# alexanderswerdlow/BEVGen

Hardware: AMD Instinct MI355X
Metric: multi-view scenes/sec (6x256x256) (higher is better)
Workload: dtype f32 (GEMM/conv/attention products as 3 f16 MFMAs on hi/lo splits, fp32 accumulate); 1 GPU; BASELINE configs[1]: Route M MaskGit, 6x256x256, batch 16 scenes/GPU, 18 iterations, + VQGAN decode to uint8; global_batch=16, parallelism=scene-parallel x1 (RCCL gather of uint8 pixels), precision_mode=f16x3

## Files before the change

### bevgen_amd/_lib.py

```python
from __future__ import annotations

import ctypes as C
import os
from typing import Optional

_HERE = os.path.dirname(os.path.abspath(__file__))
LIB_PATH = os.environ.get("BEVGEN_LIB_PATH") or os.path.join(_HERE, "csrc", "libbevgen_hip.so")
HEADER_PATH = os.path.join(os.path.dirname(_HERE), "include", "bevgen_hip.h")

ABI_VERSION = 10
ROUTE_MASKGIT, ROUTE_AR = 0, 1
PRECISION_FP32, PRECISION_BF16, PRECISION_F16X3, PRECISION_F16X1 = 0, 1, 2, 3
KV_F32, KV_F16 = 0, 1
DECODE_FUSED, DECODE_PER_OP, DECODE_SPLIT, DECODE_AUTO = 0, 1, 2, 3
VQ_OUT_RAW, VQ_OUT_DENORM, VQ_OUT_U8 = 0, 1, 2
W_F32, W_F16 = 0, 1
DTYPE_F32, DTYPE_I64, DTYPE_U8, DTYPE_F64 = 0, 1, 2, 3
ERR_NUMERIC = -5
STATUS_MLP_BARRIER, STATUS_MLP_PLACEMENT, STATUS_NONFINITE_LOGITS, STATUS_F16_RANGE, STATUS_NONFINITE_PIXELS, STATUS_NONFINITE_LATENTS = 1, 2, 4, 8, 16, 32


class BevgenError(RuntimeError):
    def __init__(self, code: int, message: str):
        super().__init__(f"libbevgen_hip error {code}: {message}")
# ... 15 lines not shown


_p = C.c_void_p
_i = C.c_int
_f = C.c_float
_l = C.c_long

SIGNATURES = {
    "bevgen_create": (_i, [C.POINTER(bevgen_cfg), _i, C.POINTER(_p)]),
    "bevgen_destroy": (None, [_p]),
    "bevgen_last_error": (C.c_char_p, [_p]),
    "bevgen_abi_version": (_i, []),
    "bevgen_synchronize": (_i, [_p, _p]),
    "bevgen_status": (_i, [_p, C.POINTER(C.c_uint)]),
    "bevgen_load_tensor": (_i, [_p, C.c_char_p, _p, _i, _i, C.POINTER(C.c_int64)]),
    "bevgen_set_tables": (_i, [_p, _p, _p, _p, _p, _p]),
    "bevgen_finalize": (_i, [_p]),
    "bevgen_muse_forward": (_i, [_p, _p, _p, _p, _p, _i, _p, _p, _p]),
    "bevgen_maskgit_generate": (_i, [_p, _p, _p, _p, _i, _i, C.POINTER(C.c_int32), _f, _i, _f, _p, _p, _p, _p, C.c_uint64, _p]),
    "bevgen_maskgit_generate_ex": (_i, [_p, _p, _p, _p, _i, _i, C.POINTER(C.c_int32), _f, _i, _f, _p, _p, _p, _p, C.c_uint64, _i, _i, _p]),
    "bevgen_op_philox_uniform": (_i, [_p, C.c_uint64, C.c_uint, C.c_uint, _i, _l, _p, _p]),
    "bevgen_sparse_self_attention": (_i, [_p, _p, _p, _p, _p, _p, _p, _i, _i, _i, _i, _p, _p]),
    "bevgen_ar_prefill": (_i, [_p, _p, _p, _p, _i, _p]),
    "bevgen_ar_logits": (_i, [_p, _p, _p]),
    "bevgen_ar_decode_step": (_i, [_p, _p, _p]),
    "bevgen_ar_forward": (_i, [_p, _p, _p, _p, _i, _p, _i, _p, _p, _p, _p, _p, _p]),
    "bevgen_ar_sample": (_i, [_p, _p, _p, _p, _i, _i, _i, _f, _i, _p, _i, _p, _p, _p]),
    "bevgen_ar_sample_forced": (_i, [_p, _p, _p, _p, _i, _i, _i, _f, _i, _p, _i, _p, _p, _p, _p]),
    "bevgen_vq_decode": (_i, [_p, _p, _i, _i, _i, _i, _p, _p]),
    "bevgen_vq_decode_latents": (_i, [_p, _p, _i, _i, _i, _i, _p, _p]),
    "bevgen_vq_encode": (_i, [_p, _p, _i, _i, _i, _p, _p]),
    "bevgen_vq_range_exponents": (_i, [_p, C.POINTER(C.c_int32), _i, C.POINTER(_i)]),
    "bevgen_op_gemm": (_i, [_p, _p, _p, _p, _p, _p, _i, _i, _i, _i, _i, _p]),
    "bevgen_op_ln_gemm": (_i, [_p, _p, _p, _p, _f, _p, _p, _p, _i, _i, _i, _i, _i, C.POINTER(_i), _p]),
    "bevgen_op_mlp_fused": (_i, [_p, _p, _p, _p, _f, _p, _p, _p, _p, _i, _p, _i, _i, _p]),
    "bevgen_op_remask": (_i, [_p, _p, _p, _p, _i, _i, _i, C.c_int64, _p]),
    "bevgen_op_maskgit_pick": (_i, [_p, _p, _p, _i, _p, _i, _i, _i, _f, C.c_int64, C.c_uint64, C.c_uint, _p, _i, _p]),
    "bevgen_op_critic_scores": (_i, [_p, _p, _i, _p, _p, _p, _f, _f, C.c_uint64, C.c_uint, _p, _i, _i, _p]),
    "bevgen_op_ar_pick": (_i, [_p, _p, _i, _p, _p, _p, _p, _i, _i, _i, _f, _p, _p, _i, _p, _p, _p, _p, _i, _i, _i, _i, _p]),
    "bevgen_op_ar_score_rows": (_i, [_p, _p, _i, _p, _p, _p, _i, _i, _i, _i, _i, _p, _p, _p]),
    "bevgen_op_mean_fixed_order": (_i, [_p, _p, _l, _p, _p]),
    "bevgen_op_layernorm": (_i, [_p, _p, _p, _p, _p, _i, _i, _f, _p]),
    "bevgen_op_geglu_layernorm": (_i, [_p, _p, _p, _p, _i, _i, _i, _p]),
    "bevgen_op_attention": (_i, [_p, _p, _p, _p, _p, _i, _i, _i, _i, _i, _f, _p, _p]),
    "bevgen_op_attention_ex": (_i, [_p, _p, _p, _p, _p, _i, _i, _i, _i, _i, _f, _i, _p, _p]),
    "bevgen_op_decode_attention": (_i, [_p, _p, _p, _p, _i, _p, _i, _p, _i, _l, _i, _i, _i, _i, _f, _p, _p]),
    "bevgen_op_ar_attn_fused": (_i, [_p, _p, _p, _i, _p, _p, _p, _p, _p, _i, _p, _p, _i, _p, _i, _p, _p, _i, _i, _i, _i, _i, _i, _i, _i, _p, _p]),
    "bevgen_op_conv3x3": (_i, [_p, _p, _p, _p, _p, _p, _i, _i, _i, _i, _i, _i, _p]),
    "bevgen_op_groupnorm": (_i, [_p, _p, _p, _p, _p, _i, _i, _i, _i, _p]),
    "bevgen_op_range_split": (_i, [_p, _p, _i, _i, _i, _p, _p, _p]),
    "bevgen_op_conv3x3_down": (_i, [_p, _p, _p, _p, _p, _i, _i, _i, _i, _i, _p]),
    "bevgen_op_vq_attn_block": (_i, [_p, _p, _p, _p, _p, _p, _p, _p, _p, _p, _p, _p, _p, _i, _i, _i, _i, _p]),
    "bevgen_op_vq_out_tail": (_i, [_p, _p, _p, _p, _p, _p, _p, _p, _i, _i, _p, _i, _i, _i, _i, _p]),
    "bevgen_op_vq_quantize": (_i, [_p, _p, _p, _p, _p, _p, _l, _i, _i, _p]),
    "bevgen_op_conv3x3_gn_stats": (_i, [_p, _p, _p, _p, _i, _p, _p, _p, _i, _i, _i, _i, _i, _p]),
    "bevgen_op_conv_ranged": (_i, [_p, _p, _p, _p, _i, _p, _p, _i, _i, _i, _i, _i, _p]),
    "bevgen_decode_attention_splits": (_i, [_i, _i, _i]),
    "bevgen_profile_begin": (_i, [_p]),
    "bevgen_profile_end": (_i, [_p, C.POINTER(C.c_double)]),
    "bevgen_ar_step_timing": (_i, [_p, _i]),
    "bevgen_ar_step_times": (_i, [_p, C.POINTER(C.c_float), _i, C.POINTER(_i)]),
    "bevgen_set_trace_buffer": (_i, [_p, _p]),
}

_lib: Optional[C.CDLL] = None

# ... 33 lines not shown
```

### bevgen_amd/csrc/api.cpp

```cpp
#include <memory>

#include "model.h"
#include "profiler.h"

using namespace bevgen;

struct bevgen_ctx : public Ctx {};

static thread_local std::string g_create_error;

template <class F>
static int guarded(bevgen_ctx* ctx, F&& f, bool check_first = true) {
    try {
        if (!ctx) return BEVGEN_ERR_INVALID;
        HIP_CHECK(hipSetDevice(ctx->device));
        split_registry_set(ctx->cfg.precision == BEVGEN_PRECISION_F16X3 ? &ctx->split : nullptr);
        struct CurrentProf {
            Profiler* old;
            unsigned* old_st;
            CurrentProf(Profiler* p, unsigned* st) : old(prof_set_current(p)), old_st(status_set_current(st)) {}
            ~CurrentProf() { prof_set_current(old); status_set_current(old_st); }
        } cur(&ctx->prof, ctx->status_dev);
        if (check_first) ctx->check_status("raised by an earlier call on this context");
        f();
// ... 260 lines not shown
            uint16_t *bp, *ap;
            ctx->arena.carve([&](Arena& ar) {
                bp = ar.get<uint16_t>((size_t)N * K * 2);
                ap = skinny >= 3 ? ar.get<uint16_t>((size_t)M * K * 2) : nullptr;
                g.kpart = skinny >= 3 && ksplit3 ? ar.get<float>((size_t)3 * M * N) : nullptr;
                g.sk_ws = skinny >= 3 && stream_k ? ar.alloc(gemm_sk_ws_bytes()) : nullptr;
            });
            launch_split_weight(w, bp, (long)N * K, (hipStream_t)stream);
            g.B_hi = bp; g.B_lo = bp + 32;
            g.a_hi_only = single;
            g.b_lo_zero = single;
            if (skinny >= 3) {
                g.b_lo_zero = skinny == 4;
                launch_split_weight(a, ap, (long)M * K, (hipStream_t)stream);
                g.A_hi = ap; g.A_lo = ap + 32;
                if (ksplit3) g.ksplit = 3;
                if (stream_k) {
                    HIP_CHECK(hipMemsetAsync(g.sk_ws, 0, 1024 * sizeof(unsigned), (hipStream_t)stream));
                    g.sk_epoch = 1; g.sk_force = true;
                }
                launch_gemm_split_glds(g, (hipStream_t)stream);
            } else {
                launch_gemm_split(g, (hipStream_t)stream);
            }
        } else if (skinny) {
            float* ws;
            ctx->arena.carve([&](Arena& ar) { ws = reinterpret_cast<float*>(ar.alloc(gemm_skinny_ws_bytes(M, N, K))); });
            launch_gemm_skinny_ws(g, ws, (hipStream_t)stream);
        }
        else launch_gemm(g, (hipStream_t)stream);
    });
}

int bevgen_op_ln_gemm(bevgen_ctx* ctx, const float* a, const float* ln_w, const float* ln_b, float eps, const float* w, const float* bias, float* c, int M, int N, int K,
                      int act_gelu, int ksplit, int* ksplit_out, void* stream) {
    return guarded(ctx, [&] {
        BG_REQUIRE(skinny_fused_supported(M, N, K, ln_w != nullptr), "op_ln_gemm: unsupported shape M=%d N=%d K=%d", M, N, K);
        SkinnyFusedArgs g;
        g.A = a; g.lda = K; g.ln_w = ln_w; g.ln_b = ln_b; g.eps = eps;
        float *wp, *cs, *ds;
        ctx->arena.carve([&](Arena& ar) {
            wp = ar.get<float>(skinny_packed_floats(N, K));
            cs = ksplit == -1 ? ar.get<float>((size_t)N) : nullptr;
            ds = ksplit == -1 ? ar.get<float>((size_t)N) : nullptr;
        });
        launch_pack_skinny_weight(w, wp, N, K, (hipStream_t)stream);
        g.Wp = wp; g.bias = bias; g.C = c; g.ldc = N;
        g.M = M; g.N = N; g.K = K; g.act = act_gelu ? ACT_GELU : ACT_NONE;
        g.ksplit = ksplit > 0 ? ksplit : (ln_w ? 1 : skinny_fused_ksplit(N, K));
        if (ksplit == -1) {
            BG_REQUIRE(ln_w && ln_b && bias, "op_ln_gemm: ksplit = -1 (folded LayerNorm) needs gamma, beta and a bias");
            launch_ar_ln_fold(w, bias, ln_w, ln_b, cs, ds, N, K, (hipStream_t)stream);
            g.ln_cs = cs; g.ln_ds = ds;
        }
        if (ksplit_out) *ksplit_out = g.ksplit;
        g.trace = ctx->trace ? ctx->trace + 4096 * 8 : nullptr;
        launch_skinny_fused(g, (hipStream_t)stream);
    });
}

int bevgen_op_mlp_fused(bevgen_ctx* ctx, const float* x, const float* ln_w, const float* ln_b, float eps, const float* w1, const float* b1, const float* w2, const float* b2,
                        int w_f16, float* out, int M, int D, void* stream) {
    return guarded(ctx, [&] {
        hipStream_t s = (hipStream_t)stream;
        BG_REQUIRE(x && ln_w && ln_b && w1 && b1 && w2 && b2 && out, "op_mlp_fused: missing operand");
        BG_REQUIRE(mlp_fused_supported(M, D, w_f16 != 0), "op_mlp_fused: unsupported shape M=%d D=%d (or a device with fewer CUs than workgroups / BEVGEN_MLP_FUSE=0)", M, D);
// ... 381 lines not shown
```

### bevgen_amd/csrc/gemm_split_glds.hip

```cpp
#include "common.h"
#include "kernels.h"
#include "profiler.h"
#include <type_traits>
#include <vector>
#include <cstdio>

namespace bevgen {

typedef _Float16 half8 __attribute__((ext_vector_type(8)));
typedef unsigned u32x4 __attribute__((ext_vector_type(4)));

struct RowDiv {
    float d, r;
    __device__ __forceinline__ explicit RowDiv(float d_) : d(d_) {
        float r0 = __builtin_amdgcn_rcpf(d_);
        const float e = fmaf(-d_, r0, 1.0f);
        r0 = fmaf(e, r0, r0);
        const float e2 = fmaf(-d_, r0, 1.0f);
        r = fmaf(e2, r0, r0);
    }
    __device__ __forceinline__ float operator()(float x) const {
        const float q0 = x * r;
        const float e = fmaf(-d, q0, x);
        return fmaf(e, r, q0);
// ... 7 lines not shown
__device__ unsigned long long g_gemm_trace[5 * 2048 * 8];
__device__ unsigned long long g_gemm_tr_tmp[2];
#define GT_STAMP(i) do { if (MODE == MODE_PLAIN && !KS) gt[i] = __builtin_amdgcn_s_memrealtime(); } while (0)
#else
#define GT_STAMP(i) do { } while (0)
#endif
constexpr float kGLoInv = 1.f / 2048.f;

__device__ __forceinline__ void glds16(const _Float16* src, _Float16* lds_wave_base) {
    __builtin_amdgcn_global_load_lds((const __attribute__((address_space(1))) void*)src, (__attribute__((address_space(3))) void*)lds_wave_base, 16, 0, 0);
}
__device__ __forceinline__ void glds16_buf(__amdgpu_buffer_rsrc_t rsrc, unsigned voff, int soff, _Float16* lds_wave_base) {
    __builtin_amdgcn_raw_ptr_buffer_load_lds(rsrc, (__attribute__((address_space(3))) void*)lds_wave_base, 16, (int)voff, soff, 0, 0);
}
template <int N>
__device__ __forceinline__ void wait_vmcnt() { asm volatile("s_waitcnt vmcnt(%0)" ::"n"(N) : "memory"); }
template <int DMA, int MAXN>
__device__ __forceinline__ void wait_tiles(int n) {
    if constexpr (MAXN <= 0) wait_vmcnt<0>();
    else {
        if (n >= MAXN) wait_vmcnt<MAXN * DMA>();
        else wait_tiles<DMA, MAXN - 1>(n);
    }
}

template <int DMA, int MAXN, int X>
__device__ __forceinline__ void wait_tiles_x(int n) {
    if constexpr (MAXN <= 0) wait_vmcnt<X>();
    else {
        if (n >= MAXN) wait_vmcnt<MAXN * DMA + X>();
        else wait_tiles_x<DMA, MAXN - 1, X>(n);
    }
}

template <int MODE, int WM, int S, bool W16, bool KS, int TI, int TJ, bool SKK = false, bool A16 = false>
__device__ __forceinline__ void gemm_tile(const GemmArgs& g, const int tx, const int ty, const int kt_first, const int nk, const int ksl, const int kz, const int sk_role,
                                          const int sk_first, const int tid
#ifdef BEVGEN_GEMM_TRACE
                                          , unsigned long long* gt
#endif
                                          ) {
    static_assert(!A16 || (W16 && MODE == MODE_PLAIN && !SKK), "single-product instantiations: rounded weight, plain GEMM, not the stream-K kernel");
    constexpr int TBM = WM * 64;
    constexpr int NW = WM * 8 / (TI * TJ);
    constexpr int WROWS = TI * 32;
    constexpr int WCOLS = TJ * 32;
    constexpr int WN = GBN / WCOLS;
    constexpr int NAJ = TBM / 8 / NW;
    constexpr int NBJ = 16 / NW;
    constexpr int AREGION = TBM * 2 * GBK;
    constexpr int STAGE_H = AREGION + GBN * 2 * GBK;
    constexpr int DMA = NAJ + NBJ;
    extern __shared__ __attribute__((aligned(1024))) _Float16 smem_g[];
    int lane = tid & 63;
    const int wave = __builtin_amdgcn_readfirstlane(tid >> 6);
    const int wm = wave / WN, wn = wave % WN;
    int r = lane & 31, h = lane >> 5;
    const int n0 = tx * GBN, m0 = ty * TBM + g.m_base;
    const int n0l = n0, m0l = m0;

    const _Float16* Ap = reinterpret_cast<const _Float16*>(g.A_hi);
    const _Float16* Bp = reinterpret_cast<const _Float16*>(g.B_hi);

    constexpr bool CONVG = MODE == MODE_CONV3, CONVS = MODE == MODE_CONV3S, CONV = CONVG || CONVS;
    unsigned a_off[NAJ], b_off[NBJ];
    int a_img[CONVG ? NAJ : 1], a_yx[CONVG ? NAJ : 1];
// ... 860 lines not shown
            if (Pp) {
                s1 += xor32(s1); s2 += xor32(s2);
                if (h == 0 && m < g.M) reinterpret_cast<float2*>(g.ln_out_stats)[(long)((n0 >> 6) + wn) * g.ln_rows + mc] = make_float2(s1, s2);
            }
        }
        if (bad) status_raise(g.status, BG_ST_F16_RANGE);
        return;
    }
    if (KS && ksl > 1) {
        float* P = g.kpart + (long)kz * g.M * g.N;
#pragma unroll
        for (int i = 0; i < TI; ++i) {
            const int m = m0 + wm * WROWS + i * 32 + r;
            if (m >= g.M) continue;
#pragma unroll
            for (int j = 0; j < 2; ++j)
#pragma unroll
                for (int qq = 0; qq < 4; ++qq) {
                    const int n = n0 + wn * 64 + j * 32 + 8 * qq + 4 * h;
#pragma unroll
                    for (int e = 0; e < 4; ++e)
                        if (n + e < g.N) P[(long)m * g.N + n + e] = accM[i][j][qq * 4 + e] + accC[i][j][qq * 4 + e] * kGLoInv;
                }
        }
        return;
    }
    }
    float* C = g.C;
    const float* Rp = g.R;
    unsigned ln_bad = 0;
    const bool vec_ok = ((g.ldc & 3) == 0) && (!Rp || (g.ldr & 3) == 0) && ((reinterpret_cast<uintptr_t>(C) & 15) == 0) &&
                        (!Rp || (reinterpret_cast<uintptr_t>(Rp) & 15) == 0);
    if constexpr (STG) {
        if (g.row_major_epi && vec_ok && (g.N & 3) == 0 && !g.ln_out_planes) {
#pragma unroll
            for (int i = 0; i < TI; ++i)
#pragma unroll
                for (int j = 0; j < TJ; ++j)
#pragma unroll
                    for (int qq = 0; qq < 4; ++qq) {
                        f32x4 v;
#pragma unroll
                        for (int e = 0; e < 4; ++e) v[e] = accM[i][j][qq * 4 + e] + accC[i][j][qq * 4 + e] * kGLoInv;
                        *reinterpret_cast<f32x4*>(pl + (i * 32 + r) * RS + j * 32 + 8 * qq + 4 * h) = v;
                    }
            constexpr int LPR = WCOLS / 4, RPP = 64 / LPR, NP = WROWS / RPP;
            const int c = lane % LPR, rr = lane / LPR;
            const int n = n0 + wn * WCOLS + 4 * c;
            const int nc = min(n, g.N - 4);
            f32x4 b4 = {0.f, 0.f, 0.f, 0.f};
            if (g.bias_n) b4 = *reinterpret_cast<const f32x4*>(g.bias_n + nc);
            f32x4 rres[NP];
            float bmr[NP];
#pragma unroll
            for (int s2 = 0; s2 < NP; ++s2) {
                const int m = min(m0 + wm * WROWS + s2 * RPP + rr, g.M - 1);
                bmr[s2] = g.bias_m ? g.bias_m[m] : 0.f;
                rres[s2] = Rp ? *reinterpret_cast<const f32x4*>(Rp + (long)m * g.ldr + nc) : f32x4{0.f, 0.f, 0.f, 0.f};
            }
#pragma unroll
            for (int s2 = 0; s2 < NP; ++s2) {
                const int row = s2 * RPP + rr, m = m0 + wm * WROWS + row;
                const f32x4 a = *reinterpret_cast<const f32x4*>(pl + row * RS + 4 * c);
                f32x4 o;
#pragma unroll
                for (int e = 0; e < 4; ++e) {
                    float t = a[e] * g.alpha + bmr[s2];
                    t += b4[e];
                    if (g.act == ACT_GELU) t = gelu_erf(t);
                    o[e] = t + rres[s2][e];
                }
                if (m < g.M && n < g.N) *reinterpret_cast<f32x4*>(C + (long)m * g.ldc + n) = o;
            }
            return;
        }
    }
    f32x4 bias4[TJ][4];
#pragma unroll
    for (int j = 0; j < TJ; ++j)
#pragma unroll
        for (int qq = 0; qq < 4; ++qq) {
            const int n = n0 + wn * WCOLS + j * 32 + 8 * qq + 4 * h;
#pragma unroll
            for (int e = 0; e < 4; ++e) bias4[j][qq][e] = (g.bias_n && n + e < g.N) ? g.bias_n[n + e] : 0.f;
        }
    f32x4 rv[TI][TJ][4];
    float bm[TI];
#pragma unroll
    for (int i = 0; i < TI; ++i) {
        const int m = min(m0 + wm * WROWS + i * 32 + r, g.M - 1);
        bm[i] = g.bias_m ? g.bias_m[m] : 0.f;
#pragma unroll
        for (int j = 0; j < TJ; ++j)
#pragma unroll
            for (int qq = 0; qq < 4; ++qq) {
                const int n = n0 + wn * WCOLS + j * 32 + 8 * qq + 4 * h;
                if (Rp && vec_ok && n + 3 < g.N) rv[i][j][qq] = *reinterpret_cast<const f32x4*>(Rp + (long)m * g.ldr + n);
                else if (Rp) {
#pragma unroll
                    for (int e = 0; e < 4; ++e) rv[i][j][qq][e] = Rp[(long)m * g.ldr + min(n + e, g.N - 1)];
                } else rv[i][j][qq] = f32x4{0.f, 0.f, 0.f, 0.f};
            }
    }
#pragma unroll
    for (int i = 0; i < TI; ++i) {
// ... 219 lines not shown
```

### bevgen_amd/csrc/muse.cpp

```cpp
#include "model.h"
#include "muse_plan.h"

namespace bevgen {

namespace {

struct MuseWs {
    int B = 0;
    int S = 1;
    bool generate = false;

    long rows = 0;
    float *img = nullptr, *c_embed = nullptr, *context = nullptr;
    int64_t* cond_g = nullptr; float* c_embed_g = nullptr;
    std::vector<float*> crossK, crossV;
    float *logits = nullptr, *scores = nullptr;
    float *x = nullptr, *xn = nullptr, *qraw = nullptr, *kvraw = nullptr, *Q = nullptr, *Ks = nullptr, *Vs = nullptr, *att = nullptr, *h = nullptr, *g = nullptr;
    size_t kvS = 0, kvC = 0;
    float* attn_ws = nullptr; int attn_ks = 1;
    float* kpart = nullptr;
    float *stats_d = nullptr, *stats_f = nullptr;
    float* rowstat = nullptr;
    void* sk_ws = nullptr;
    unsigned sk_epoch = 0;
    const float *token_emb = nullptr, *pos_emb = nullptr, *norm_g = nullptr, *to_logits = nullptr, *critic_w = nullptr, *critic_b = nullptr;
};

MuseSwitches muse_switches() {
    static const MuseSwitches once = [] {
        const auto env = [](const char* name, int dflt) { const char* v = getenv(name); return v ? atoi(v) : dflt; };
        MuseSwitches s;
        s.qkv_merge = env("BEVGEN_QKV_MERGE", 1);
        s.qkv_wm4 = env("BEVGEN_QKV_WM4", 1);
        s.ksplit = env("BEVGEN_KSPLIT", 0);
        s.attn_ksplit = env("BEVGEN_ATTN_KSPLIT", 0);
        return s;
    }();
    MuseSwitches s = once;
    const char *fold = getenv("BEVGEN_LN_FOLD"), *merge = getenv("BEVGEN_LN_MERGE");
    s.ln_fold = fold ? atoi(fold) : 1;
    s.ln_merge = merge ? (merge[0] == 't' ? 1 : 0) : -1;
    return s;
}

struct Planes { _Float16 *hi, *lo; };
Planes planes_of(float* buf, size_t n) { _Float16* hi = reinterpret_cast<_Float16*>(buf); return {hi, hi + n}; }

struct In { const float* p = nullptr; int ld = 0; };
struct Out { float* p = nullptr; int ld = 0; };

GemmArgs gemm_args(const Ctx& c, In W, Out C, int M, int N, int K, In R = {}) {
    GemmArgs g;
    g.B = W.p; g.C = C.p; g.R = R.p;
    g.M = M; g.N = N; g.K = K;
    g.ldb = W.ld; g.ldc = C.ld; g.ldr = R.ld;
    g.a_hi_only = c.single_product;
    return g;
}
void gemm(In A, GemmArgs g, hipStream_t s) {
    g.A = A.p; g.lda = A.ld;
    launch_gemm(g, s);
}
GemmArgs on_planes(const void* planes, int lda, GemmArgs g) {
    g.A_hi = reinterpret_cast<const uint16_t*>(planes); g.A_lo = g.A_hi + 32;
    g.lda = lda;
    return g;
}

struct LnFold {
    const float* in_stats = nullptr; const float* in_cs = nullptr;
    const float* in_gsums = nullptr; int in_groups = 0, in_count = 0;
    void* out_planes = nullptr; float* out_stats = nullptr; int out_ld = 0;
};
// ... 112 lines not shown
    sa.bias = c.bias_cross; sa.bias_pk = c.bias_cross_pk; sa.ldbias = c.ldC;
    sa.kv_group = w.S;
    launch_attention_split(sa, f.s);
    project(f, PROJ_OUT, on_planes(w.att, D, gemm_args(c, {l.to_out[1], D}, {w.x, D}, rows, D, D, {w.x, D})), f.fold == 2 ? &f.prod_x : nullptr);
}

void feed_forward_split(Fwd& f, const MuseLayer& l, bool last) {
    const Ctx& c = f.c;
    MuseWs& w = f.w;
    const int D = c.D, rows = f.rows, fold = f.fold;
    if (fold != 2) launch_layernorm_planes(w.x, D, l.ff_g0, nullptr, w.xn, D, rows, D, 1e-5f, f.s);
    if (l.ff_w1_geglu) {
        GemmArgs ge = on_planes(w.xn, D, gemm_args(c, {fold == 2 ? l.fold_w1 : l.ff_w1_geglu, D}, {w.h, c.Fpad}, rows, 2 * c.Fpad, D));
        ge.epi = EPI_GEGLU;
        LnFold fg;
        if (fold == 2) fg = consumer(f, w.stats_d, D / 32, D, l.fold_w1_cs);
        if (fold >= 1) { fg.out_planes = w.g; fg.out_stats = w.stats_f; fg.out_ld = c.Fpad; }
        project(f, PROJ_GEGLU, ge, fold >= 1 ? &fg : nullptr);
        if (fold == 0) launch_layernorm_planes(w.h, c.Fpad, l.ff_g3, nullptr, w.g, c.Fpad, rows, c.F, 1e-5f, f.s);
    } else {
        project(f, PROJ_UP, on_planes(w.xn, D, gemm_args(c, {l.ff_w1, D}, {w.h, 2 * c.F}, rows, 2 * c.F, D)));
        launch_geglu_layernorm_planes(w.h, 2 * c.F, l.ff_g3, w.g, c.Fpad, rows, c.F, 1e-5f, f.s);
    }
    LnFold fd;
    if (fold >= 1 && l.ff_w1_geglu) fd = consumer(f, w.stats_f, c.Fpad / 32, c.F, l.fold_w4_cs);
    const bool prod_next = fold == 2 && !last;
    if (prod_next) { fd.out_planes = w.xn; fd.out_stats = w.stats_d; fd.out_ld = D; }
    const bool cons = fd.in_stats || fd.in_gsums, any = cons || fd.out_planes;
    project(f, PROJ_OUT, on_planes(w.g, c.Fpad, gemm_args(c, {cons ? l.fold_w4 : l.ff_w4_padded, c.Fpad}, {w.x, D}, rows, D, c.Fpad, {w.x, D})), any ? &fd : nullptr);
    f.x_planes_ready = prod_next;
}

void muse_blocks_split(const Ctx& c, MuseWs& w, hipStream_t s) {
    Fwd f{c, w, s, (int)w.rows, w.B, c.N, muse_switches()};
    f.fold = muse_fold_level(f.sw, !c.muse.empty() && c.muse[0].fold_w4);
    f.tile_merge = muse_tile_merge(f.sw, f.rows);
    f.prod_x.out_planes = w.xn; f.prod_x.out_stats = w.stats_d; f.prod_x.out_ld = c.D;
    const int layers = c.cfg.num_layers;
    for (int i = 0; i < layers; ++i) {
        const MuseLayer& l = c.muse[i];
        self_attention_split(f, l);
        cross_attention_split(f, l, i);
        feed_forward_split(f, l, i + 1 == layers);
    }
}

void muse_blocks_f32(const Ctx& c, MuseWs& w, hipStream_t s) {
    const int D = c.D, H = c.H, B = w.B, N = c.N, F = c.F, Fpad = c.Fpad, rows = (int)w.rows;
    AttnArgs self{};
    self.Q = w.Q; self.K = w.Ks; self.V = w.Vs; self.bias = c.bias_self; self.R = nullptr; self.O = w.att;
    self.B = B; self.H = H; self.Nq = N; self.Nk_pad = c.NkS_pad;
    self.q_bstride = (long)H * N * 64; self.q_hstride = (long)N * 64;
    self.kv_bstride = (long)H * c.NkS_pad * 64; self.kv_hstride = (long)c.NkS_pad * 64;
    self.ldbias = c.ldS; self.bias_head_stride = 0; self.scale = 8.0f;
    self.o_bstride = (long)N * D; self.o_qstride = D; self.o_hstride = 64;
    AttnArgs cross = self;
    cross.bias = c.bias_cross; cross.Nk_pad = c.NkC_pad; cross.ldbias = c.ldC;
    cross.kv_bstride = (long)H * c.NkC_pad * 64; cross.kv_hstride = (long)c.NkC_pad * 64;
    cross.kv_group = w.S;
    for (int i = 0; i < c.cfg.num_layers; ++i) {
        const MuseLayer& l = c.muse[i];
        launch_layernorm(w.x, D, l.norm_g[0], nullptr, w.xn, D, rows, D, 1e-5f, s);
        gemm({w.xn, D}, gemm_args(c, {l.to_q[0], D}, {w.qraw, D}, rows, D, D), s);
        gemm({w.xn, D}, gemm_args(c, {l.to_kv[0], D}, {w.kvraw, 2 * D}, rows, 2 * D, D), s);
        launch_muse_q_prep(w.qraw, l.q_scale[0], w.Q, B, H, N, s);
        launch_muse_kv_prep(w.kvraw, l.null_kv[0], l.k_scale[0], w.Ks, w.Vs, B, H, N, c.NkS_pad, s);
        launch_attention(self, s);
        gemm({w.att, D}, gemm_args(c, {l.to_out[0], D}, {w.x, D}, rows, D, D, {w.x, D}), s);
        launch_layernorm(w.x, D, l.norm_g[1], nullptr, w.xn, D, rows, D, 1e-5f, s);
        gemm({w.xn, D}, gemm_args(c, {l.to_q[1], D}, {w.qraw, D}, rows, D, D), s);
        launch_muse_q_prep(w.qraw, l.q_scale[1], w.Q, B, H, N, s);
        cross.K = w.crossK[i]; cross.V = w.crossV[i];
        launch_attention(cross, s);
        gemm({w.att, D}, gemm_args(c, {l.to_out[1], D}, {w.x, D}, rows, D, D, {w.x, D}), s);
        launch_layernorm(w.x, D, l.ff_g0, nullptr, w.xn, D, rows, D, 1e-5f, s);
        gemm({w.xn, D}, gemm_args(c, {l.ff_w1, D}, {w.h, 2 * F}, rows, 2 * F, D), s);
        launch_geglu_layernorm(w.h, 2 * F, l.ff_g3, w.g, Fpad, rows, F, 1e-5f, s);
        gemm({w.g, Fpad}, gemm_args(c, {l.ff_w4_padded, Fpad}, {w.x, D}, rows, D, Fpad, {w.x, D}), s);
    }
}

void muse_layout(const Ctx& c, MuseWs& w, Arena& a) {
    const auto& g = c.cfg;
    const MuseSwitches sw = muse_switches();
    const int D = c.D, H = c.H, B = w.B, G = B / w.S;
    w.img = g.image_embed ? a.get<float>((size_t)w.rows * D) : nullptr;
    w.c_embed = g.image_embed ? a.get<float>((size_t)B * g.num_cams * D) : nullptr;
    w.context = a.get<float>((size_t)G * c.K * D);
    w.x = a.get<float>((size_t)w.rows * D);
    w.xn = a.get<float>((size_t)w.rows * D);
    w.qraw = a.get<float>((size_t)w.rows * D);
    w.att = a.get<float>((size_t)w.rows * D);
    w.kvraw = a.get<float>((size_t)std::max<long>(w.rows, (long)B * c.K) * 2 * D);
    w.Q = a.get<float>((size_t)w.rows * D);
    w.kvS = (size_t)B * H * c.NkS_pad * 64;
    w.Ks = a.get<float>(w.kvS);
    w.Vs = a.get<float>(w.kvS);
    w.h = a.get<float>((size_t)w.rows * 2 * c.F);
    w.g = a.get<float>((size_t)w.rows * c.Fpad);
    w.kpart = muse_needs_kpart(w.rows, D, c.Fpad, sw) ? a.get<float>((size_t)kMuseKsplitMax * w.rows * D) : nullptr;
    w.attn_ks = pick_attn_ksplit((long)cdiv(c.N, 256) * H * B, c.NkS_pad / 32, sw.attn_ksplit);
    w.attn_ws = w.attn_ks > 1 ? a.get<float>((size_t)attn_split_ws_floats(B, H, c.N, w.attn_ks)) : nullptr;
    w.stats_d = a.get<float>((size_t)w.rows * 2 * (D / 32));
    w.stats_f = a.get<float>((size_t)w.rows * 2 * (c.Fpad / 32));
    w.rowstat = a.get<float>((size_t)w.rows * 2);
    w.sk_ws = w.rows <= kMuseSkMaxRows && g.precision == BEVGEN_PRECISION_F16X3 ? a.alloc(gemm_sk_ws_bytes()) : nullptr;
    w.cond_g = w.S > 1 ? a.get<int64_t>((size_t)G * c.K) : nullptr;
    w.c_embed_g = w.S > 1 && g.image_embed ? a.get<float>((size_t)G * g.num_cams * D) : nullptr;
    w.kvC = (size_t)G * H * c.NkC_pad * 64;
    w.crossK.resize(g.num_layers);
    w.crossV.resize(g.num_layers);
    for (int i = 0; i < g.num_layers; ++i) {
        w.crossK[i] = a.get<float>(w.kvC);
        w.crossV[i] = a.get<float>(w.kvC);
    }
    w.logits = w.generate ? a.get<float>((size_t)w.rows * c.V) : nullptr;
    w.scores = w.generate ? a.get<float>((size_t)w.rows) : nullptr;
// ... 109 lines not shown
```

### bevgen_amd/csrc/muse_plan.h

```cpp
#pragma once
#include "gemm_plan.h"

namespace bevgen {

struct MuseSwitches {
    int ln_fold = 1;
    int ln_merge = -1;
    int qkv_merge = 1;
    int qkv_wm4 = 1;
    int ksplit = 0;
    int attn_ksplit = 0;
};

inline int muse_fold_level(const MuseSwitches& sw, bool has_fold_constants) { return has_fold_constants ? std::max(0, std::min(sw.ln_fold, 2)) : 0; }

inline bool muse_tile_merge(const MuseSwitches& sw, long rows) { return sw.ln_merge >= 0 ? sw.ln_merge == 1 : rows <= 3072; }

inline bool muse_qkv_merged(const MuseSwitches& sw, long rows) { return sw.qkv_merge != 0 && (sw.qkv_merge != 3 || rows <= 3072); }

constexpr int kMuseKsplitMax = 6;
inline int pick_ksplit(long rows, int N, int K, int ksplit_switch) {
    if ((long)cdiv(rows, 256) * cdiv(N, 128) >= 256) return 1;
    const long tiles = (long)cdiv(rows, 128) * cdiv(N, 128);
    if (tiles >= 160) return 1;
    int s = (K >= 2048 && tiles > 128) ? 2 : 1;
    if (ksplit_switch > 0) s = std::min(kMuseKsplitMax, ksplit_switch);
    while (s > 1 && K / 32 < 2 * s) --s;
    return s;
}
inline bool muse_needs_kpart(long rows, int D, int Fpad, const MuseSwitches& sw) { return std::max(pick_ksplit(rows, D, D, sw.ksplit), pick_ksplit(rows, D, Fpad, sw.ksplit)) > 1; }

inline int pick_attn_ksplit(long blocks, int ntiles, int attn_ksplit_switch) {
    if (attn_ksplit_switch > 0) return std::max(1, std::min(std::min(attn_ksplit_switch, 8), ntiles));
    if (blocks * 2 > 256) return 1;
    const int ks = std::min(std::min(4, (int)(256 / blocks)), ntiles / 8);
    return std::max(ks, 1);
}

constexpr long kMuseSkMaxRows = 8192;

enum MuseProj { PROJ_OUT = 0, PROJ_Q = 1, PROJ_KV = 2, PROJ_GEGLU = 3, PROJ_UP = 4 };
struct MuseProjIn {
    MuseProj kind = PROJ_UP;
    long M = 0; int N = 0, K = 0;
    bool fold_role = false;
    bool merged = false;
    bool has_kpart = false;
// ... 30 lines not shown
```

### bevgen_amd/runtime.py

```python
from __future__ import annotations

import ctypes as C
import os
import math
from typing import Dict, Mapping, Optional, Sequence

import numpy as np
import torch

from . import _lib, tables
from ._lib import bevgen_cfg
from .weights import ff_inner_dim


def _ptr(t: Optional[torch.Tensor]):
    return None if t is None else C.c_void_p(t.data_ptr())


def _stream(device=None):
    return C.c_void_p(torch.cuda.current_stream(device).cuda_stream)


def _req(t: torch.Tensor, dtype, device, name: str) -> torch.Tensor:
    if t.dtype != dtype:
# ... 349 lines not shown
    def profile_begin(self):
        self._check(self.lib.bevgen_profile_begin(self._h))

    def profile_end(self) -> Dict[str, Dict[str, float]]:
        buf = (C.c_double * (3 * len(self.PROFILE_KINDS)))()
        self._check(self.lib.bevgen_profile_end(self._h, buf))
        return {k: {"launches": buf[3 * i], "ms": buf[3 * i + 1], "work": buf[3 * i + 2]} for i, k in enumerate(self.PROFILE_KINDS)}

    def ar_step_timing(self, enable: bool = True):
        self._check(self.lib.bevgen_ar_step_timing(self._h, int(enable)))

    def ar_step_times(self, cap: int = 4096):
        buf = (C.c_float * cap)()
        n = C.c_int(0)
        self._check(self.lib.bevgen_ar_step_times(self._h, buf, cap, C.byref(n)))
        return np.frombuffer(buf, dtype=np.float32, count=n.value).copy()

    def trace_begin(self):
        self._trace = torch.zeros((3, 4096, 8), dtype=torch.int64, device=self.device)
        self._check(self.lib.bevgen_set_trace_buffer(self._h, _ptr(self._trace)))

    def trace_end(self):
        torch.cuda.synchronize()
        self._check(self.lib.bevgen_set_trace_buffer(self._h, None))
        return self._trace.cpu()

    def op_gemm(self, a, w, bias=None, residual=None, gelu=False, skinny=False):
        M, K = a.shape
        N = w.shape[0]
        c = torch.empty((M, N), dtype=torch.float32, device=self.device)
        self._check(self.lib.bevgen_op_gemm(self._h, _ptr(a), _ptr(w), _ptr(bias), _ptr(residual), _ptr(c), M, N, K, int(gelu), int(skinny), self._s()))
        return c

    def op_ln_gemm(self, a, w, ln_w=None, ln_b=None, bias=None, gelu=False, ksplit=0, eps=1e-5):
        M, K = a.shape
        N = w.shape[0]
        ks = C.c_int(0)
        out = torch.empty((4, M, N), dtype=torch.float32, device=self.device)
        self._check(self.lib.bevgen_op_ln_gemm(self._h, _ptr(a), _ptr(ln_w), _ptr(ln_b), float(eps), _ptr(w), _ptr(bias), _ptr(out), M, N, K, int(gelu), int(ksplit),
                                               C.byref(ks), self._s()))
        return out[0] if ks.value == 1 else out[:ks.value].sum(0)

    def op_mlp_fused(self, x, ln_w, ln_b, w1, b1, w2, b2, w_f16=False, eps=1e-5):
        M, D = x.shape
        out = torch.empty((M, D), dtype=torch.float32, device=self.device)
        self._check(self.lib.bevgen_op_mlp_fused(self._h, _ptr(x), _ptr(ln_w), _ptr(ln_b), float(eps), _ptr(w1), _ptr(b1), _ptr(w2), _ptr(b2), int(w_f16), _ptr(out), M, D, self._s()))
        return out

    @staticmethod
    def _ld(t, ld):
        assert t.dim() == 2 and (t.shape[1] == 1 or t.stride(1) == 1), "rows must be unit-stride"
        return int(ld) if ld is not None else (t.stride(0) if t.shape[0] > 1 else t.shape[1])

    def op_remask(self, ids, scores, n_mask, mask_id, init_ids=None):
        rows, T = ids.shape
        self._check(self.lib.bevgen_op_remask(self._h, _ptr(ids), _ptr(scores), _ptr(init_ids), rows, T, int(n_mask), int(mask_id), self._s()))
        return ids

    def op_maskgit_pick(self, ids, logits, V, *, mask_id, k=None, topk_filter_thres=None, temperature=1.0, gumbel_u=None, seed=0, it=0, conf_scores=None, conf_mode=0, ldl=None):
        if k is None:
            k = V if topk_filter_thres is None else topk_count(topk_filter_thres, V)
        self._check(self.lib.bevgen_op_maskgit_pick(self._h, _ptr(ids), _ptr(logits), self._ld(logits, ldl), _ptr(gumbel_u), ids.numel(), int(V), int(k), float(temperature),
                                                    int(mask_id), C.c_uint64(int(seed) & 0xFFFFFFFFFFFFFFFF), int(it), _ptr(conf_scores), int(conf_mode), self._s()))
        return ids

    def op_critic_scores(self, embed, w, b, D=None, *, u=None, noise_scale=0.0, frac=0.0, seed=0, it=0, lde=None):
# ... 149 lines not shown
```

### include/bevgen_hip.h

```cpp
#ifndef BEVGEN_HIP_H
#define BEVGEN_HIP_H

#include <stddef.h>
#include <stdint.h>

#ifdef __cplusplus
extern "C" {
#endif

#define BEVGEN_ABI_VERSION 10

enum { BEVGEN_ROUTE_MASKGIT = 0, BEVGEN_ROUTE_AR = 1 };
enum { BEVGEN_PRECISION_FP32 = 0, BEVGEN_PRECISION_BF16 = 1 , BEVGEN_PRECISION_F16X3 = 2, BEVGEN_PRECISION_F16X1 = 3 };
enum { BEVGEN_KV_F32 = 0, BEVGEN_KV_F16 = 1 };
enum { BEVGEN_DECODE_FUSED = 0, BEVGEN_DECODE_PER_OP = 1, BEVGEN_DECODE_SPLIT = 2, BEVGEN_DECODE_AUTO = 3 };
enum { BEVGEN_W_F32 = 0, BEVGEN_W_F16 = 1 };
enum { BEVGEN_DTYPE_F32 = 0, BEVGEN_DTYPE_I64 = 1, BEVGEN_DTYPE_U8 = 2, BEVGEN_DTYPE_F64 = 3 };

enum {
    BEVGEN_OK = 0,
    BEVGEN_ERR_INVALID = -1,
    BEVGEN_ERR_HIP = -2,
    BEVGEN_ERR_STATE = -3,
    BEVGEN_ERR_INTERNAL = -4,
// ... 68 lines not shown

int bevgen_sparse_self_attention(bevgen_ctx* ctx, const float* d_q, const float* d_k, const float* d_v, const int64_t* d_layout,
                                 const float* d_attn_mask, const float* d_add_mask, int B, int H, int L, int block, float* d_out, void* stream);

int bevgen_ar_prefill(bevgen_ctx* ctx, const int64_t* d_cond_ids, const float* d_I_inv, const float* d_E_inv, int B, void* stream);

int bevgen_ar_logits(bevgen_ctx* ctx, float* d_logits, void* stream);

int bevgen_ar_decode_step(bevgen_ctx* ctx, const int64_t* d_token, void* stream);

int bevgen_ar_forward(bevgen_ctx* ctx, const int64_t* d_cond_ids, const float* d_I_inv, const float* d_E_inv, int B, const int64_t* d_ids, int n_steps,
                      float* d_logits, const int64_t* d_target, const float* d_weight, float* d_nll, float* d_loss, void* stream);

int bevgen_ar_sample(bevgen_ctx* ctx, const int64_t* d_cond_ids, const float* d_I_inv, const float* d_E_inv, int B, int steps,
                     int top_k, float temperature, int greedy, const float* d_noise_u, int samples_per_layout,
                     int64_t* d_out_ids, float* d_step_logits , void* stream);

int bevgen_ar_sample_forced(bevgen_ctx* ctx, const int64_t* d_cond_ids, const float* d_I_inv, const float* d_E_inv, int B, int steps,
                            int top_k, float temperature, int greedy, const float* d_noise_u, int samples_per_layout,
                            const int64_t* d_forced_ids, int64_t* d_out_ids, float* d_step_logits, void* stream);


enum { BEVGEN_VQ_OUT_RAW = 0, BEVGEN_VQ_OUT_DENORM = 1, BEVGEN_VQ_OUT_U8 = 2 };
int bevgen_vq_decode(bevgen_ctx* ctx, const int64_t* d_ids, int n, int lat_h, int lat_w, int out_mode, void* d_out, void* stream);

int bevgen_vq_encode(bevgen_ctx* ctx, const float* d_x, int n, int H, int W, int64_t* d_ids, void* stream);

int bevgen_vq_decode_latents(bevgen_ctx* ctx, const float* d_zq, int n, int lat_h, int lat_w, int out_mode, void* d_out, void* stream);

int bevgen_vq_range_exponents(bevgen_ctx* ctx, int32_t* h_out, int cap, int* count);

int bevgen_op_gemm(bevgen_ctx* ctx, const float* d_a, const float* d_w, const float* d_bias, const float* d_residual, float* d_c,
                   int M, int N, int K, int act_gelu, int skinny, void* stream);
int bevgen_op_ln_gemm(bevgen_ctx* ctx, const float* d_a, const float* d_ln_w, const float* d_ln_b, float eps, const float* d_w, const float* d_bias, float* d_c,
                      int M, int N, int K, int act_gelu, int ksplit, int* ksplit_out, void* stream);
int bevgen_op_mlp_fused(bevgen_ctx* ctx, const float* d_x, const float* d_ln_w, const float* d_ln_b, float eps, const float* d_w1 , const float* d_b1,
                        const float* d_w2 , const float* d_b2, int w_f16, float* d_out, int M, int D, void* stream);
int bevgen_op_philox_uniform(bevgen_ctx* ctx, unsigned long long seed, unsigned iter, unsigned stream_id, int V , long n,
                             float* d_out, void* stream);
int bevgen_op_remask(bevgen_ctx* ctx, int64_t* d_ids, const float* d_scores, const int64_t* d_init_ids , int rows, int T, int n_mask, int64_t mask_id, void* stream);
int bevgen_op_maskgit_pick(bevgen_ctx* ctx, int64_t* d_ids, const float* d_logits, int ldl, const float* d_gumbel_u , int rows, int V, int k, float temperature,
                           int64_t mask_id, unsigned long long seed, unsigned iter, float* d_conf_scores , int conf_mode, void* stream);
int bevgen_op_critic_scores(bevgen_ctx* ctx, const float* d_embed, int lde, const float* d_w, const float* d_b, const float* d_u , float noise_scale, float frac,
                            unsigned long long seed, unsigned iter, float* d_scores, int rows, int D, void* stream);
int bevgen_op_ar_pick(bevgen_ctx* ctx, const float* d_logits, int ldl, const float* d_u , const int* d_step , const int64_t* d_forced ,
                      int64_t* d_out, int rows, int V, int top_k, float temperature, int64_t* d_out_all , const int64_t* d_fwd_idx, int N, const float* d_tok_emb,
                      const float* d_img_embed , const float* d_pos_emb, float* d_x , int C, int T, int D, int vocab_rows, void* stream);
int bevgen_op_ar_score_rows(bevgen_ctx* ctx, const float* d_logits, int ldl, const int64_t* d_target , const float* d_weight ,
                            const int64_t* d_fwd_idx, int b, int s0, int rows, int N, int V, float* d_nll , float* d_wnll, void* stream);
int bevgen_op_mean_fixed_order(bevgen_ctx* ctx, const float* d_x, long n, float* d_out, void* stream);
int bevgen_op_layernorm(bevgen_ctx* ctx, const float* d_x, const float* d_gamma, const float* d_beta, float* d_y, int rows, int D, float eps, void* stream);
int bevgen_op_geglu_layernorm(bevgen_ctx* ctx, const float* d_h, const float* d_gamma, float* d_y, int rows, int F, int ldy, void* stream);
int bevgen_op_attention(bevgen_ctx* ctx, const float* d_q, const float* d_k, const float* d_v, const float* d_bias, int ldbias,
                        int B, int H, int Nq, int Nk_pad, float scale, float* d_out, void* stream);
int bevgen_op_attention_ex(bevgen_ctx* ctx, const float* d_q, const float* d_k, const float* d_v, const float* d_bias, int ldbias,
                           int B, int H, int Nq, int Nk_pad, float scale, int key_splits, float* d_out, void* stream);
int bevgen_op_decode_attention(bevgen_ctx* ctx, const float* d_q, const void* d_kcache, const void* d_vcache, int kv_dtype,
                               const float* d_bias, int ldbias, const uint8_t* d_keep, int ldkeep, long keep_head_stride,
                               int B, int H, int n, int Lmax, float scale, float* d_out, void* stream);
int bevgen_op_ar_attn_fused(bevgen_ctx* ctx, const float* d_x, const float* d_partial, int ns, const float* d_rbias, const float* d_ln_w, const float* d_ln_b,
                            const float* d_wqkv, const float* d_bqkv, int w_f16, void* d_kcache, void* d_vcache, int kv_dtype, const float* d_bias, int ldbias,
                            const float* d_attn_mask, const int64_t* d_layout, int block, int B, int G, int H, int n, int Lmax, int prefix, int split, float* d_out, void* stream);
int bevgen_op_conv3x3(bevgen_ctx* ctx, const float* d_x_nhwc, const float* d_w_ohwi, const float* d_bias, const float* d_residual,
                      float* d_y_nhwc, int n, int H, int W, int Cin, int Cout, int upsample2x, void* stream);
int bevgen_op_groupnorm(bevgen_ctx* ctx, const float* d_x_nhwc, const float* d_gamma, const float* d_beta, float* d_y, int n, int hw, int C,
                        int swish, void* stream);
// ... 31 lines not shown
```

Baseline: 11.16 scenes/s.

## Emit LayerNorm-fold f16 planes and row stats from row-major GEMM epilogue

The row-major vectorized GEMM epilogue can now produce the next layer's f16 hi/lo split planes and per-32-column sum/sumsq statistics while storing the fp32 output, using DPP cross-lane reductions and lane swaps. Previously that path was skipped whenever LN output planes were requested. The default LN fold level becomes 2 when the row count is at most 3072, so the fused fold path is active for the MaskGit batch. The aim is to remove a separate LayerNorm/split pass over activations, at the cost of a heavier epilogue and more register pressure. A test entry point is also added.

```diff
diff --git a/bevgen_amd/_lib.py b/bevgen_amd/_lib.py
--- a/bevgen_amd/_lib.py
+++ b/bevgen_amd/_lib.py
@@ -71,6 +71,7 @@
     "bevgen_vq_encode": (_i, [_p, _p, _i, _i, _i, _p, _p]),
     "bevgen_vq_range_exponents": (_i, [_p, C.POINTER(C.c_int32), _i, C.POINTER(_i)]),
     "bevgen_op_gemm": (_i, [_p, _p, _p, _p, _p, _p, _i, _i, _i, _i, _i, _p]),
+    "bevgen_op_gemm_ln_fold": (_i, [_p, _p, _p, _p, _p, _p, _p, _p, _i, _i, _i, _i, _p]),
     "bevgen_op_ln_gemm": (_i, [_p, _p, _p, _p, _f, _p, _p, _p, _i, _i, _i, _i, _i, C.POINTER(_i), _p]),
     "bevgen_op_mlp_fused": (_i, [_p, _p, _p, _p, _f, _p, _p, _p, _p, _i, _p, _i, _i, _p]),
     "bevgen_op_remask": (_i, [_p, _p, _p, _p, _i, _i, _i, C.c_int64, _p]),
diff --git a/bevgen_amd/csrc/api.cpp b/bevgen_amd/csrc/api.cpp
--- a/bevgen_amd/csrc/api.cpp
+++ b/bevgen_amd/csrc/api.cpp
@@ -316,6 +316,29 @@
     });
 }
 
+int bevgen_op_gemm_ln_fold(bevgen_ctx* ctx, const float* a, const float* w, float* c, void* planes, float* stats, const float* in_stats, const float* in_cs, int M, int N, int K,
+                           int w_f16, void* stream) {
+    return guarded(ctx, [&] {
+        BG_REQUIRE(a && w && c && planes && stats && (!in_stats || in_cs), "op_gemm_ln_fold: bad arguments");
+        GemmArgs g;
+        g.B = w; g.C = c; g.R = c;
+        g.M = M; g.N = N; g.K = K; g.lda = K; g.ldb = K; g.ldc = N; g.ldr = N;
+        g.ln_out_planes = planes; g.ln_out_stats = stats; g.ln_out_ld = N; g.ln_rows = M;
+        g.ln_in_stats = in_stats; g.ln_in_cs = in_cs;
+        uint16_t *bp, *ap;
+        ctx->arena.carve([&](Arena& ar) {
+            bp = ar.get<uint16_t>((size_t)N * K * 2);
+            ap = ar.get<uint16_t>((size_t)M * K * 2);
+        });
+        launch_split_weight(w, bp, (long)N * K, (hipStream_t)stream);
+        launch_split_weight(a, ap, (long)M * K, (hipStream_t)stream);
+        g.B_hi = bp; g.B_lo = bp + 32;
+        g.A_hi = ap; g.A_lo = ap + 32;
+        g.b_lo_zero = w_f16 != 0;
+        launch_gemm_split_glds(g, (hipStream_t)stream);
+    });
+}
+
 int bevgen_op_ln_gemm(bevgen_ctx* ctx, const float* a, const float* ln_w, const float* ln_b, float eps, const float* w, const float* bias, float* c, int M, int N, int K,
                       int act_gelu, int ksplit, int* ksplit_out, void* stream) {
     return guarded(ctx, [&] {
diff --git a/bevgen_amd/csrc/gemm_split_glds.hip b/bevgen_amd/csrc/gemm_split_glds.hip
--- a/bevgen_amd/csrc/gemm_split_glds.hip
+++ b/bevgen_amd/csrc/gemm_split_glds.hip
@@ -63,6 +63,9 @@
         else wait_tiles_x<DMA, MAXN - 1, X>(n);
     }
 }
+
+template <int N>
+__device__ __forceinline__ float row_shr(float x) { return __int_as_float(__builtin_amdgcn_mov_dpp(__float_as_int(x), 0x110 + N, 0xf, 0xf, true)); }
 
 template <int MODE, int WM, int S, bool W16, bool KS, int TI, int TJ, bool SKK = false, bool A16 = false>
 __device__ __forceinline__ void gemm_tile(const GemmArgs& g, const int tx, const int ty, const int kt_first, const int nk, const int ksl, const int kz, const int sk_role,
@@ -989,7 +992,9 @@
     const bool vec_ok = ((g.ldc & 3) == 0) && (!Rp || (g.ldr & 3) == 0) && ((reinterpret_cast<uintptr_t>(C) & 15) == 0) &&
                         (!Rp || (reinterpret_cast<uintptr_t>(Rp) & 15) == 0);
     if constexpr (STG) {
-        if (g.row_major_epi && vec_ok && (g.N & 3) == 0 && !g.ln_out_planes) {
+        if (g.row_major_epi && vec_ok && (g.N & 3) == 0) {
+            const bool prod = g.ln_out_planes != nullptr;
+            _Float16* const Pp = reinterpret_cast<_Float16*>(g.ln_out_planes);
 #pragma unroll
             for (int i = 0; i < TI; ++i)
 #pragma unroll
@@ -1015,6 +1020,8 @@
                 bmr[s2] = g.bias_m ? g.bias_m[m] : 0.f;
                 rres[s2] = Rp ? *reinterpret_cast<const f32x4*>(Rp + (long)m * g.ldr + nc) : f32x4{0.f, 0.f, 0.f, 0.f};
             }
+            const auto passes = [&](auto prod_c) {
+            constexpr bool PROD = decltype(prod_c)::value;
 #pragma unroll
             for (int s2 = 0; s2 < NP; ++s2) {
                 const int row = s2 * RPP + rr, m = m0 + wm * WROWS + row;
@@ -1027,7 +1034,40 @@
                     if (g.act == ACT_GELU) t = gelu_erf(t);
                     o[e] = t + rres[s2][e];
                 }
-                if (m < g.M && n < g.N) *reinterpret_cast<f32x4*>(C + (long)m * g.ldc + n) = o;
+                const bool inside = m < g.M && n < g.N;
+                if (inside) *reinterpret_cast<f32x4*>(C + (long)m * g.ldc + n) = o;
+                if constexpr (PROD) {
+                    const float p1 = (o[0] + o[1]) + (o[2] + o[3]);
+                    const float p2 = fmaf(o[0], o[0], o[1] * o[1]) + fmaf(o[2], o[2], o[3] * o[3]);
+                    float t1 = 0.f + p1, t2 = 0.f + p2;
+#pragma unroll
+                    for (int st = 0; st < 3; ++st) { t1 = row_shr<2>(t1) + p1; t2 = row_shr<2>(t2) + p2; }
+                    t1 += row_shr<1>(t1); t2 += row_shr<1>(t2);
+                    if ((c & 7) == 7) *reinterpret_cast<float2*>(pl + row * RS + WCOLS + 2 * (c >> 3)) = make_float2(t1, t2);
+                    half4_t hi4, lo4;
+#pragma unroll
+                    for (int e = 0; e < 4; ++e) { hi4[e] = split_hi(o[e]); lo4[e] = split_lo(o[e], hi4[e]); }
+                    if (inside) guard_half4(hi4, ln_bad);
+                    const bool odd = c & 1;
+                    const uint2 hw = __builtin_bit_cast(uint2, hi4), lw = __builtin_bit_cast(uint2, lo4);
+                    const uint2 send = odd ? hw : lw;
+                    const uint2 recv = make_uint2((unsigned)__builtin_amdgcn_mov_dpp((int)send.x, 0xB1, 0xf, 0xf, true), (unsigned)__builtin_amdgcn_mov_dpp((int)send.y, 0xB1, 0xf, 0xf, true));
+                    const uint4 pk = odd ? make_uint4(recv.x, recv.y, lw.x, lw.y) : make_uint4(hw.x, hw.y, recv.x, recv.y);
+                    if (inside) *reinterpret_cast<uint4*>(Pp + (long)m * 2 * g.ln_out_ld + (n >> 5) * 64 + 8 * ((c & 7) >> 1) + (odd ? 32 : 0)) = pk;
+                }
+            }
+            };
+            if (!prod) { passes(std::false_type{}); return; }
+            passes(std::true_type{});
+            {
+#pragma unroll
+                for (int it = 0; it < (WROWS * TJ + 63) / 64; ++it) {
+                    const int idx = it * 64 + lane, j = idx / WROWS, row = idx % WROWS;
+                    const int m = m0 + wm * WROWS + row, grp = (n0 + wn * WCOLS + j * 32) >> 5;
+                    if (idx < WROWS * TJ && m < g.M && grp * 32 < g.N)
+                        reinterpret_cast<float2*>(g.ln_out_stats)[(long)grp * g.ln_rows + m] = *reinterpret_cast<const float2*>(pl + row * RS + WCOLS + 2 * j);
+                }
+                if (ln_bad) status_raise(g.status, BG_ST_F16_RANGE);
             }
             return;
         }
diff --git a/bevgen_amd/csrc/muse.cpp b/bevgen_amd/csrc/muse.cpp
--- a/bevgen_amd/csrc/muse.cpp
+++ b/bevgen_amd/csrc/muse.cpp
@@ -26,7 +26,7 @@
     const float *token_emb = nullptr, *pos_emb = nullptr, *norm_g = nullptr, *to_logits = nullptr, *critic_w = nullptr, *critic_b = nullptr;
 };
 
-MuseSwitches muse_switches() {
+MuseSwitches muse_switches(long rows) {
     static const MuseSwitches once = [] {
         const auto env = [](const char* name, int dflt) { const char* v = getenv(name); return v ? atoi(v) : dflt; };
         MuseSwitches s;
@@ -38,7 +38,7 @@
     }();
     MuseSwitches s = once;
     const char *fold = getenv("BEVGEN_LN_FOLD"), *merge = getenv("BEVGEN_LN_MERGE");
-    s.ln_fold = fold ? atoi(fold) : 1;
+    s.ln_fold = fold ? atoi(fold) : muse_default_fold(rows);
     s.ln_merge = merge ? (merge[0] == 't' ? 1 : 0) : -1;
     return s;
 }
@@ -217,7 +217,7 @@
 }
 
 void muse_blocks_split(const Ctx& c, MuseWs& w, hipStream_t s) {
-    Fwd f{c, w, s, (int)w.rows, w.B, c.N, muse_switches()};
+    Fwd f{c, w, s, (int)w.rows, w.B, c.N, muse_switches(w.rows)};
     f.fold = muse_fold_level(f.sw, !c.muse.empty() && c.muse[0].fold_w4);
     f.tile_merge = muse_tile_merge(f.sw, f.rows);
     f.prod_x.out_planes = w.xn; f.prod_x.out_stats = w.stats_d; f.prod_x.out_ld = c.D;
@@ -267,7 +267,7 @@
 
 void muse_layout(const Ctx& c, MuseWs& w, Arena& a) {
     const auto& g = c.cfg;
-    const MuseSwitches sw = muse_switches();
+    const MuseSwitches sw = muse_switches(w.rows);
     const int D = c.D, H = c.H, B = w.B, G = B / w.S;
     w.img = g.image_embed ? a.get<float>((size_t)w.rows * D) : nullptr;
     w.c_embed = g.image_embed ? a.get<float>((size_t)B * g.num_cams * D) : nullptr;
diff --git a/bevgen_amd/csrc/muse_plan.h b/bevgen_amd/csrc/muse_plan.h
--- a/bevgen_amd/csrc/muse_plan.h
+++ b/bevgen_amd/csrc/muse_plan.h
@@ -13,6 +13,8 @@
 };
 
 inline int muse_fold_level(const MuseSwitches& sw, bool has_fold_constants) { return has_fold_constants ? std::max(0, std::min(sw.ln_fold, 2)) : 0; }
+constexpr long kMuseFold2MaxRows = 3072;
+inline int muse_default_fold(long rows) { return rows <= kMuseFold2MaxRows ? 2 : 1; }
 
 inline bool muse_tile_merge(const MuseSwitches& sw, long rows) { return sw.ln_merge >= 0 ? sw.ln_merge == 1 : rows <= 3072; }
 
diff --git a/bevgen_amd/runtime.py b/bevgen_amd/runtime.py
--- a/bevgen_amd/runtime.py
+++ b/bevgen_amd/runtime.py
@@ -405,6 +405,15 @@
         self._check(self.lib.bevgen_op_gemm(self._h, _ptr(a), _ptr(w), _ptr(bias), _ptr(residual), _ptr(c), M, N, K, int(gelu), int(skinny), self._s()))
         return c
 
+    def op_gemm_ln_fold(self, a, w, x, in_stats=None, in_cs=None, w_f16=False):
+        M, K = a.shape
+        N = w.shape[0]
+        c = x.clone()
+        planes = torch.zeros((M, N // 32, 2, 32), dtype=torch.float16, device=self.device)
+        stats = torch.zeros((N // 32, M, 2), dtype=torch.float32, device=self.device)
+        self._check(self.lib.bevgen_op_gemm_ln_fold(self._h, _ptr(a), _ptr(w), _ptr(c), _ptr(planes), _ptr(stats), _ptr(in_stats), _ptr(in_cs), M, N, K, int(w_f16), self._s()))
+        return c, planes, stats
+
     def op_ln_gemm(self, a, w, ln_w=None, ln_b=None, bias=None, gelu=False, ksplit=0, eps=1e-5):
         M, K = a.shape
         N = w.shape[0]
diff --git a/include/bevgen_hip.h b/include/bevgen_hip.h
--- a/include/bevgen_hip.h
+++ b/include/bevgen_hip.h
@@ -124,6 +124,8 @@
 
 int bevgen_op_gemm(bevgen_ctx* ctx, const float* d_a, const float* d_w, const float* d_bias, const float* d_residual, float* d_c,
                    int M, int N, int K, int act_gelu, int skinny, void* stream);
+int bevgen_op_gemm_ln_fold(bevgen_ctx* ctx, const float* d_a, const float* d_w, float* d_c, void* d_planes, float* d_stats, const float* d_in_stats ,
+                           const float* d_in_cs , int M, int N, int K, int w_f16, void* stream);
 int bevgen_op_ln_gemm(bevgen_ctx* ctx, const float* d_a, const float* d_ln_w, const float* d_ln_b, float eps, const float* d_w, const float* d_bias, float* d_c,
                       int M, int N, int K, int act_gelu, int ksplit, int* ksplit_out, void* stream);
 int bevgen_op_mlp_fused(bevgen_ctx* ctx, const float* d_x, const float* d_ln_w, const float* d_ln_b, float eps, const float* d_w1 , const float* d_b1,
```

After: 11.16 scenes/s, median of 2. No clear change (+0.0%).
